# xxxupeng/stereo_toolbox

Hardware: AMD Instinct MI355X
Metric: stereo pairs/sec @ 540x960 D=192 (GwcNet_GC fwd+bwd) (higher is better)
Workload: dtype f32; 1 GPU; GwcNet_GC(maxdisp=192) train step: fwd+bwd+allreduce+Adam, 576x960 pairs (reference pad_to_2x shape), batch 1/GPU, fp32, synthetic randn inputs, deterministic filler weights; global_batch=1, parallelism=dp1, grad_sync=none (single rank: flat fp32 buffer packed, no collective), launch=eager, optimizer=torch.optim.Adam(fused=True)

## Files before the change

### include/stx_hip.h

```cpp
#ifndef STX_HIP_H
#define STX_HIP_H
#ifdef __cplusplus
extern "C" {
#endif

const char* stx_last_error(void);
const char* stx_build_info(void);
int stx_get_tuning(const char* name);
int stx_set_tuning(const char* name, int value);

int stx_cost_volume_fwd(const float* Lg, const float* Rg, int Cg, int G, const float* Lc, const float* Rc, int Cc,
                        const float* scale, float* vol, int B, int H, int W, int D, int mask_left, void* stream);
int stx_group_normalize_fwd(const float* x, float* y, int B, int C, int G, int HW, float out_scale, void* stream);
int stx_group_normalize_bwd(const float* x, const float* gy, float* gx, int B, int C, int G, int HW, float out_scale, void* stream);
int stx_cost_volume_bwd(const float* gvol, const float* Lg, const float* Rg, int Cg, int G, int Cc, float* gLg,
                        float* gRg, float* gLc, float* gRc, int B, int H, int W, int D, int mask_left, void* stream);

int stx_head_fwd(const float* cost, float* disp, float* stats, int B, int Dc, int Hc, int Wc, int D, int H, int W,
                 void* stream);
long long stx_head_bwd_workspace_floats(int B, int Dc, int H, int W);
int stx_head_bwd(const float* gdisp, const float* cost, const float* disp, const float* stats, float* gcost,
                 float* workspace, int B, int Dc, int Hc, int Wc, int D, int H, int W, void* stream);
int stx_head_fwd2(const float* cost, float* disp, float* stats, int B, int Dc, int Hc, int Wc, int D, int H, int W,
                  int align_corners, void* stream);
// ... 27 lines not shown
int stx_conv3d_wgrad_bn(const float* x, const float* gy, const float* z, const float* scale, const float* shift, const float* mean,
                        const float* invstd, const float* gamma, const float* sums, float inv_n, int act, float* dz, float* dw,
                        float* workspace, int B, int D, int H, int W, int CF, int CC, void* stream);

int stx_conv2d_supported(int Cin, int Cout);
long long stx_conv2d_stat_rows(int groups);
int stx_conv2d_fwd(const float* x, const float* w, float* out, float* stats, int B, int H, int W, int Cin, int Cout, int dgrad,
                   int groups, void* stream);

int stx_conv3d_c1_fwd(const float* x, const float* w, const float* residual, float* out, int B, int D, int H, int W,
                      int Cin, void* stream);
long long stx_conv3d_c1_wgrad_workspace_floats(int Cin);
int stx_conv3d_c1_wgrad(const float* x, const float* gy, float* dw, float* workspace, int B, int D, int H, int W,
                        int Cin, void* stream);
int stx_conv3d_c1_dgrad(const float* gy, const float* w, float* gx, int B, int D, int H, int W, int Cin, void* stream);

int stx_mish_fwd(const float* x, float* y, long long n, void* stream);
int stx_mish_bwd(const float* gy, const float* x, float* gx, long long n, void* stream);
int stx_depth_to_space(const float* y, float* out, int B, int D, int H, int W, int C, int inverse, void* stream);
int stx_gate_fwd(const float* cv, const float* att, float* out, int B, int D, long long HW, int C, void* stream);
int stx_gate_bwd(const float* g, const float* cv, const float* att, float* gcv, float* gatt, int B, int D, long long HW,
                 int C, void* stream);

int stx_concat_channels(const float* in0, const float* in1, const float* in2, const float* in3, int C0, int C1, int C2, int C3,
                        float* out, long long nvox, void* stream);
int stx_split_channels(const float* in, float* out0, float* out1, float* out2, float* out3, int C0, int C1, int C2, int C3,
                       long long nvox, void* stream);
int stx_transpose(const float* in, float* out, int N, int rows, int cols, void* stream);

int stx_dwconv_hw_fwd(const float* x, const float* w, const int* dil, float* out, int B, int D, int H, int W, int C,
// ... 175 lines not shown
```

### stereo_toolbox_amd/_capi.py

```python
import ctypes
import os
import threading

import torch

_P = ctypes.c_void_p
_I = ctypes.c_int
_F = ctypes.c_float
_L = ctypes.c_longlong

SIGNATURES = {
    "stx_get_tuning": [ctypes.c_char_p],
    "stx_set_tuning": [ctypes.c_char_p, _I],
    "stx_cost_volume_fwd": [_P, _P, _I, _I, _P, _P, _I, _P, _P, _I, _I, _I, _I, _I, _P],
    "stx_cost_volume_bwd": [_P, _P, _P, _I, _I, _I, _P, _P, _P, _P, _I, _I, _I, _I, _I, _P],
    "stx_group_normalize_fwd": [_P, _P, _I, _I, _I, _I, _F, _P],
    "stx_group_normalize_bwd": [_P, _P, _P, _I, _I, _I, _I, _F, _P],
    "stx_head_fwd": [_P, _P, _P, _I, _I, _I, _I, _I, _I, _I, _P],
    "stx_head_bwd_workspace_floats": [_I, _I, _I, _I],
    "stx_head_bwd": [_P, _P, _P, _P, _P, _P, _I, _I, _I, _I, _I, _I, _I, _P],
    "stx_head_fwd2": [_P, _P, _P, _I, _I, _I, _I, _I, _I, _I, _I, _P],
    "stx_head_bwd2": [_P, _P, _P, _P, _P, _P, _I, _I, _I, _I, _I, _I, _I, _I, _P],
    "stx_softargmax_fwd": [_P, _P, _I, _I, _I, _P],
    "stx_argmax_fwd": [_P, _P, _I, _I, _I, _P],
# ... 9 lines not shown
    "stx_conv3d_fwd_stat_rows": [_I, _I, _I, _I, _I, _I, _I, _I],
    "stx_deconv3d_fwd_blocks": [_I, _I, _I],
    "stx_conv3d_fwd": [_P, _P, _P, _P, _P, _P, _P, _I, _I, _I, _I, _I, _I, _I, _I, _I, _P],
    "stx_deconv3d_fwd": [_P, _P, _P, _P, _P, _P, _P, _I, _I, _I, _I, _I, _I, _I, _I, _I, _I, _P],
    "stx_conv3d_wgrad_workspace_floats": [_I, _I, _I, _I, _I, _I, _I, _I],
    "stx_conv3d_wgrad": [_P, _P, _P, _P, _I, _I, _I, _I, _I, _I, _I, _I, _I, _I, _I, _P],
    "stx_conv3d_wgrad_bn_supported": [_I, _I, _I, _I, _I, _I],
    "stx_conv3d_wgrad_bn": [_P] * 9 + [_F, _I, _P, _P, _P, _I, _I, _I, _I, _I, _I, _P],
    "stx_conv2d_supported": [_I, _I],
    "stx_conv2d_stat_rows": [_I],
    "stx_conv2d_fwd": [_P, _P, _P, _P, _I, _I, _I, _I, _I, _I, _I, _P],
    "stx_conv3d_c1_fwd": [_P, _P, _P, _P, _I, _I, _I, _I, _I, _P],
    "stx_conv3d_c1_wgrad_workspace_floats": [_I],
    "stx_conv3d_c1_wgrad": [_P, _P, _P, _P, _I, _I, _I, _I, _I, _P],
    "stx_conv3d_c1_dgrad": [_P, _P, _P, _I, _I, _I, _I, _I, _P],
    "stx_mish_fwd": [_P, _P, _L, _P],
    "stx_mish_bwd": [_P, _P, _P, _L, _P],
    "stx_depth_to_space": [_P, _P, _I, _I, _I, _I, _I, _I, _P],
    "stx_gate_fwd": [_P, _P, _P, _I, _I, _L, _I, _P],
    "stx_gate_bwd": [_P, _P, _P, _P, _P, _I, _I, _L, _I, _P],
    "stx_concat_channels": [_P, _P, _P, _P, _I, _I, _I, _I, _P, _L, _P],
    "stx_split_channels": [_P, _P, _P, _P, _P, _I, _I, _I, _I, _L, _P],
    "stx_transpose": [_P, _P, _I, _I, _I, _P],
    "stx_dwconv_hw_fwd": [_P, _P, _P, _P, _I, _I, _I, _I, _I, _I, _P],
    "stx_dwconv_hw_wgrad_workspace_floats": [_I],
    "stx_dwconv_hw_wgrad": [_P, _P, _P, _P, _P, _I, _I, _I, _I, _I, _P],
    "stx_cost_volume_scale_bwd": [_P, _P, _P, _P, _I, _I, _I, _I, _I, _I, _P],
    "stx_scale_channels": [_P, _P, _P, _L, _I, _P],
    "stx_ac_volume_bwd": [_P, _P, _P, _P, _P, _P, _P, _I, _I, _I, _I, _I, _I, _P],
    "stx_pad_normalize_u8": [_P, _P, _I, _I, _I, _I, _I, _I, _P, _P, _P],
# ... 144 lines not shown
```

### stereo_toolbox_amd/aggregation.py

```python
import os
import threading

import torch
import torch.nn as nn

from . import ops


def _is_transposed(conv):
    return isinstance(conv, nn.ConvTranspose3d)


def _conv_cfg(conv):
    ks = conv.kernel_size[0]
    stride = conv.stride[0]
    if _is_transposed(conv):
        k3 = ks == 3 and stride == 2 and conv.padding[0] == 1 and conv.output_padding[0] == 1
        k4 = ks == 4 and stride == 2 and conv.padding[0] == 1 and conv.output_padding[0] == 0
        if not (k3 or k4) or len(set(conv.kernel_size)) != 1 or len(set(conv.stride)) != 1:
            raise ops.StxError("only ConvTranspose3d(k=3, s=2, p=1, op=1) and ConvTranspose3d(k=4, s=2, p=1) are on the hot path")
    else:
        if not ((ks == 3 and conv.padding[0] == 1 and stride in (1, 2)) or (ks == 1 and conv.padding[0] == 0 and stride == 1)):
            raise ops.StxError(f"unsupported Conv3d k={ks} s={stride} p={conv.padding}")
    if conv.bias is not None or conv.groups != 1:
# ... 164 lines not shown
    if bn is None:
        y = z1
        if residual is not None:
            y = y + residual
        if relu == 3:
            return torch.nn.functional.leaky_relu(y, 0.01)
        return torch.relu(y) if relu else y
    count1 = z1.numel() // z1.shape[-1]
    st1 = _bn_state(bn, part1 if want else None, count1)
    if second is not None:
        x2, conv2, bn2 = second
        want2 = bn2.training
        z2, part2 = second_raw if second_raw is not None else _raw_conv(x2, conv2, want2)
        st2 = _bn_state(bn2, part2 if want2 else None, z2.numel() // z2.shape[-1])
        return ops.BnActFn.apply(z1, bn.weight, bn.bias, z2, bn2.weight, bn2.bias, None, relu, st1, st2)
    defer = (residual is None and want and relu in (0, 1, False, True) and not _is_transposed(conv) and _conv_cfg(conv) == (3, 1)
             and conv.weight.shape[0] % 32 == 0 and conv.weight.shape[1] % 32 == 0 and not st1.get("sync")
             and os.environ.get("STX_BN_BWD_IN_WGRAD", "1") != "0")
    if defer:
        ops.bn_defer_reset_if_stale()
    return ops.BnActFn.apply(z1, bn.weight, bn.bias, None, None, None, residual, relu, st1, None, 1, defer)


@ops.fp32_region
def convbn_block(x, seq, relu=False, second=None, residual=None, mish=False, raw=None, second_raw=None):
    sec = None
    if second is not None:
        sec = (second[0], second[1][0], second[1][1])
    return conv_block(x, seq[0], seq[1], relu=relu, second=sec, residual=residual, mish=mish, raw=raw, second_raw=second_raw)
```

### stereo_toolbox_amd/csrc/conv_c1.hip

```cpp
#include "stx_common.h"
#include <stdlib.h>

namespace {

constexpr int C1_THREADS = 256;
constexpr int C1_TD = 2, C1_TH = 4, C1_TW = 32;
constexpr int C1_ED = C1_TD + 2, C1_EH = C1_TH + 2, C1_EW = C1_TW + 2;
constexpr int C1_CK = 16, C1_VS = C1_CK + 4;

struct C1Args {
    const float* x;
    const float* w;
    const float* gy;
    const float* res;
    float* out;
    int B, D, H, W, Cin;
    int nDt, nHt, nWt, ntiles;
};

__device__ __forceinline__ void c1_stage(const C1Args& a, float* tile, int b, int d0, int h0, int w0, int c0, int tid) {
    for (int idx = tid; idx < C1_ED * C1_EH * C1_EW * (C1_CK / 4); idx += C1_THREADS) {
        const int v = idx / (C1_CK / 4), f = idx - v * (C1_CK / 4);
        const int wx = v % C1_EW, hy = (v / C1_EW) % C1_EH, dz = v / (C1_EW * C1_EH);
        const int gd = d0 - 1 + dz, gh = h0 - 1 + hy, gw = w0 - 1 + wx;
// ... 228 lines not shown
        const unsigned vbase = (unsigned)((((oh < H ? oh : 0) * W + w0 + 4 * half) * 32 + i) * 4);
#pragma unroll
        for (int r = 0; r < 16; ++r) {
            const int m = (r & 3) + 8 * (r >> 2);
            const bool ok = oh < H && w0 + 4 * half + m < W;
            stx_buf_st1(ors, ok ? vbase : STX_BUF_OOB, (unsigned)(m * 128), acc[r]);
        }
    }
}


constexpr int C1M_TD = 2, C1M_TH = 8, C1M_TW = 32;
constexpr int C1M_ED = C1M_TD + 2, C1M_EH = C1M_TH + 2, C1M_EW = C1M_TW + 2;
constexpr int C1M_BLOCKS = 1024;

__global__ __launch_bounds__(C1_THREADS) void conv_c1_wgrad_mfma_kernel(const float* __restrict__ x,
                                                                        const float* __restrict__ gy,
                                                                        float* __restrict__ slab, int B, int D, int H,
                                                                        int W, int Cin, int nDt, int nHt, int nWt,
                                                                        int ntiles) {
    __shared__ float gys[C1M_ED * C1M_EH * C1M_EW];
    __shared__ float red[4][1024];
    const int tid = threadIdx.x, lane = tid & 63, wave = tid >> 6;
    const int i = lane & 31, half = lane >> 5;
    const int cb = blockIdx.y;
    const int kd = i / 9, kh = (i / 3) % 3, kw = i % 3;
    const int toff = (i < 27) ? ((2 - kd) * C1M_EH + (2 - kh)) * C1M_EW + (2 - kw) + half : half;
    f32x16 acc;
#pragma unroll
    for (int r = 0; r < 16; ++r) acc[r] = 0.f;
    for (int t = blockIdx.x; t < ntiles; t += gridDim.x) {
        int r = t;
        const int wt = r % nWt; r /= nWt;
        const int ht = r % nHt; r /= nHt;
        const int dt = r % nDt;
        const int b = r / nDt;
        const int d0 = dt * C1M_TD, h0 = ht * C1M_TH, w0 = wt * C1M_TW;
        __syncthreads();
        for (int idx = tid; idx < C1M_ED * C1M_EH * C1M_EW; idx += C1_THREADS) {
            const int wx = idx % C1M_EW, hy = (idx / C1M_EW) % C1M_EH, dz = idx / (C1M_EW * C1M_EH);
            const int gd = d0 - 1 + dz, gh = h0 - 1 + hy, gw = w0 - 1 + wx;
            gys[idx] = (gd >= 0 && gd < D && gh >= 0 && gh < H && gw >= 0 && gw < W)
                           ? gy[(((size_t)b * D + gd) * H + gh) * W + gw] : 0.f;
        }
        __syncthreads();
#pragma unroll 1
        for (int k = 0; k < 4; ++k) {
            const int row = wave * 4 + k;
            const int ld = row / C1M_TH, lh = row % C1M_TH;
            const int gd = d0 + ld, gh = h0 + lh;
            const bool rowok = gd < D && gh < H;
            const float* xr = x + ((((size_t)b * D + gd) * H + gh) * W + w0 + half) * Cin + cb * 32 + i;
            float av[16];
#pragma unroll
            for (int p = 0; p < 16; ++p)
                av[p] = (rowok && w0 + 2 * p + half < W) ? xr[(size_t)(2 * p) * Cin] : 0.f;
            const float* gp = gys + (ld * C1M_EH + lh) * C1M_EW + toff;
#pragma unroll
            for (int p = 0; p < 16; ++p) {
                float bv = gp[2 * p];
                bv = (i < 27) ? bv : 0.f;
                acc = __builtin_amdgcn_mfma_f32_32x32x2f32(av[p], bv, acc, 0, 0, 0);
            }
        }
    }
#pragma unroll
    for (int r = 0; r < 16; ++r) red[wave][((r & 3) + 8 * (r >> 2) + 4 * half) * 32 + i] = acc[r];
    __syncthreads();
    float* dst = slab + ((size_t)cb * gridDim.x + blockIdx.x) * 1024;
    for (int idx = tid; idx < 1024; idx += C1_THREADS)
        dst[idx] = (red[0][idx] + red[1][idx]) + (red[2][idx] + red[3][idx]);
// ... 10 lines not shown
    red[tid] = s;
    __syncthreads();
    for (int k = C1_THREADS / 2; k > 0; k >>= 1) {
        if (tid < k) red[tid] += red[tid + k];
        __syncthreads();
    }
    if (tid == 0) dw[m] = (float)red[0];
}


constexpr int C1F_TH = 8, C1F_TW = 32;
constexpr int C1F_EH = C1F_TH + 2, C1F_EW = C1F_TW + 2, C1F_NV = C1F_EH * C1F_EW;
constexpr int C1F_MT = (C1F_NV + 31) / 32;
constexpr int C1F_WGS = 512;

__global__ __launch_bounds__(C1_THREADS) void conv_c1_fwd_mfma_kernel(const float* __restrict__ x,
                                                                      const float* __restrict__ w,
                                                                      const float* __restrict__ res,
                                                                      float* __restrict__ out, int B, int D, int H, int W,
                                                                      int nHt, int nWt, int ncols) {
    STX_DYN_SMEM(smem);
    float* Ps = reinterpret_cast<float*>(smem);
    const int tid = threadIdx.x, lane = tid & 63, wave = __builtin_amdgcn_readfirstlane(tid >> 6);
    const int i = lane & 31, half = lane >> 5;
    float wreg[16];
#pragma unroll
    for (int s_ = 0; s_ < 16; ++s_) wreg[s_] = (i < 27) ? w[(size_t)(16 * half + s_) * 27 + i] : 0.f;
    const int lh = tid / C1F_TW, lw = tid % C1F_TW;

    constexpr int MTW = (C1F_MT + 3) / 4;
    const long long units = (long long)ncols * D;
    int u = __builtin_amdgcn_readfirstlane((int)(units * blockIdx.x / gridDim.x));
    const int u_end = __builtin_amdgcn_readfirstlane((int)(units * (blockIdx.x + 1) / gridDim.x));
    const unsigned plane_bytes = (unsigned)H * (unsigned)W * 32u * 4u;
    while (u < u_end) {
        const int col = u / D;
        const int d_lo = u - col * D;
        const int left = u_end - u;
        const int d_hi = (D - d_lo < left) ? D : d_lo + left;
        u += d_hi - d_lo;
        const int wt = col % nWt, ht = (col / nWt) % nHt, b = col / (nWt * nHt);
        const int h0 = ht * C1F_TH, w0 = wt * C1F_TW;
// ... 22 lines not shown
        __syncthreads();
        for (int p = d_lo - 1; p <= d_hi; ++p) {
            float* Pb = Ps + ((p + 2) & 1) * (C1F_NV * 27);
            const bool pin = p >= 0 && p < D;
            float4 cur[MTW][4];
#pragma unroll
            for (int t = 0; t < MTW; ++t)
#pragma unroll
                for (int q = 0; q < 4; ++q) cur[t][q] = nxt[t][q];
            load_plane(p + 1);
            if (pin) {
#pragma unroll
                for (int t = 0; t < MTW; ++t) {
                    const int m = wave + 4 * t;
                    if (m < C1F_MT) {
                        f32x16 acc;
#pragma unroll
                        for (int r = 0; r < 16; ++r) acc[r] = 0.f;
#pragma unroll
                        for (int q = 0; q < 4; ++q) {
                            acc = __builtin_amdgcn_mfma_f32_32x32x2f32(cur[t][q].x, wreg[4 * q + 0], acc, 0, 0, 0);
                            acc = __builtin_amdgcn_mfma_f32_32x32x2f32(cur[t][q].y, wreg[4 * q + 1], acc, 0, 0, 0);
                            acc = __builtin_amdgcn_mfma_f32_32x32x2f32(cur[t][q].z, wreg[4 * q + 2], acc, 0, 0, 0);
                            acc = __builtin_amdgcn_mfma_f32_32x32x2f32(cur[t][q].w, wreg[4 * q + 3], acc, 0, 0, 0);
                        }
                        if (i < 27) {
#pragma unroll
                            for (int r = 0; r < 16; ++r) {
                                const int v = m * 32 + (r & 3) + 8 * (r >> 2) + 4 * half;
                                if (v < C1F_NV) Pb[v * 27 + i] = acc[r];
// ... 17 lines not shown
            }
            const float done = accA + s2;
            const int od = p - 1;
            if (od >= d_lo && od < d_hi && ook) {
                const size_t o = (((size_t)b * D + od) * H + oh) * W + ow;
                out[o] = res ? done + res[o] : done;
            }
            accA = accB + s1;
            accB = s0;
        }
    }
}

}

extern "C" int stx_conv3d_c1_fwd(const float* x, const float* w, const float* residual, float* out, int B, int D,
                                 int H, int W, int Cin, void* stream) {
    stx_begin();
    STX_REQUIRE(x && w && out && B > 0 && D > 0 && H > 0 && W > 0, "conv3d_c1_fwd: bad shape");
    STX_REQUIRE(Cin % C1_CK == 0, "conv3d_c1_fwd: Cin=%d must be a multiple of %d", Cin, C1_CK);
    if (Cin == 32 && (long long)H * W * 128 < (1ll << 31)) {
        const int nHt = stx_cdiv(H, C1F_TH), nWt = stx_cdiv(W, C1F_TW);
        const long long ncols = (long long)B * nHt * nWt, units = ncols * D;
        STX_REQUIRE(units < (1ll << 31), "conv3d_c1_fwd: volume too large");
        long long g = C1F_WGS;
        if (g > units / 4) g = units / 4 > 0 ? units / 4 : 1;
        const size_t lds = (size_t)2 * C1F_NV * 27 * 4;
        if (int rc = stx_lds_require((const void*)conv_c1_fwd_mfma_kernel, lds, "conv3d_c1_fwd(mfma)")) return rc;
        hipLaunchKernelGGL(conv_c1_fwd_mfma_kernel, dim3((unsigned)g), dim3(C1_THREADS), lds, (hipStream_t)stream, x, w,
                           residual, out, B, D, H, W, nHt, nWt, (int)ncols);
        return stx_check_launch("conv3d_c1_fwd(mfma)");
    }
    C1Args a;
    a.x = x; a.w = w; a.gy = nullptr; a.res = residual; a.out = out;
    a.B = B; a.D = D; a.H = H; a.W = W; a.Cin = Cin;
    a.nDt = stx_cdiv(D, C1_TD); a.nHt = stx_cdiv(H, C1_TH); a.nWt = stx_cdiv(W, C1_TW);
    a.ntiles = B * a.nDt * a.nHt * a.nWt;
    if (int rc = stx_lds_require((const void*)conv_c1_fwd_kernel, C1_TILE_BYTES, "conv3d_c1_fwd")) return rc;
    hipLaunchKernelGGL(conv_c1_fwd_kernel, dim3(a.ntiles), dim3(C1_THREADS), C1_TILE_BYTES, (hipStream_t)stream, a);
    return stx_check_launch("conv3d_c1_fwd");
}

extern "C" long long stx_conv3d_c1_wgrad_workspace_floats(int Cin) {
    const long long valu = (long long)C1_WGRAD_BLOCKS * Cin * 27;
    const long long mfma = (long long)C1M_BLOCKS * 1024 * ((Cin + 31) / 32);
    return valu > mfma ? valu : mfma;
}

extern "C" int stx_conv3d_c1_wgrad(const float* x, const float* gy, float* dw, float* workspace, int B, int D, int H,
                                   int W, int Cin, void* stream) {
    stx_begin();
    STX_REQUIRE(x && gy && dw && workspace && B > 0, "conv3d_c1_wgrad: null operand");
    STX_REQUIRE(Cin % C1_CK == 0 && Cin <= 4 * C1_CK, "conv3d_c1_wgrad: Cin=%d must be 16..64 in steps of 16", Cin);
    if (Cin % 32 == 0) {
        const int nDt = stx_cdiv(D, C1M_TD), nHt = stx_cdiv(H, C1M_TH), nWt = stx_cdiv(W, C1M_TW);
        const long long nt = (long long)B * nDt * nHt * nWt;
        STX_REQUIRE(nt < (1ll << 31), "conv3d_c1_wgrad: volume too large");
        const int nblk = nt < C1M_BLOCKS ? (int)nt : C1M_BLOCKS;
        hipStream_t st = (hipStream_t)stream;
        hipLaunchKernelGGL(conv_c1_wgrad_mfma_kernel, dim3(nblk, Cin / 32), dim3(C1_THREADS), 0, st, x, gy, workspace, B,
                           D, H, W, Cin, nDt, nHt, nWt, (int)nt);
        int rc = stx_check_launch("conv3d_c1_wgrad(mfma)");
        if (rc) return rc;
        hipLaunchKernelGGL(c1m_reduce_kernel, dim3(Cin * 27), dim3(C1_THREADS), 0, st, workspace, nblk, dw);
        return stx_check_launch("conv3d_c1_wgrad(reduce)");
    }
    C1Args a;
    a.x = x; a.w = nullptr; a.gy = gy; a.res = nullptr; a.out = workspace;
    a.B = B; a.D = D; a.H = H; a.W = W; a.Cin = Cin;
    a.nDt = stx_cdiv(D, C1_TD); a.nHt = stx_cdiv(H, C1_TH); a.nWt = stx_cdiv(W, C1_TW);
    a.ntiles = B * a.nDt * a.nHt * a.nWt;
    const int nblk = a.ntiles < C1_WGRAD_BLOCKS ? a.ntiles : C1_WGRAD_BLOCKS;
    const size_t lds = C1_TILE_BYTES + 256 * 4;
    hipStream_t st = (hipStream_t)stream;
    if (int rc = stx_lds_require((const void*)conv_c1_wgrad_kernel, lds, "conv3d_c1_wgrad")) return rc;
    hipLaunchKernelGGL(conv_c1_wgrad_kernel, dim3(nblk), dim3(C1_THREADS), lds, st, a);
    if (int rc = stx_check_launch("conv3d_c1_wgrad")) return rc;
    hipLaunchKernelGGL(c1_colsum_kernel, dim3(Cin * 27), dim3(C1_THREADS), 0, st, workspace, nblk, Cin * 27, dw);
    return stx_check_launch("conv3d_c1_colsum");
}

extern "C" int stx_conv3d_c1_dgrad(const float* gy, const float* w, float* gx, int B, int D, int H, int W, int Cin,
                                   void* stream) {
    stx_begin();
    STX_REQUIRE(gy && w && gx && B > 0 && D > 0 && H > 0 && W > 0, "conv3d_c1_dgrad: bad shape");
    STX_REQUIRE(Cin % 4 == 0 && Cin <= 64, "conv3d_c1_dgrad: Cin=%d must be a multiple of 4, <= 64", Cin);
    const int nHt = stx_cdiv(H, C1D_TH), nWt = stx_cdiv(W, C1D_TW);
    const long long nt = (long long)B * D * nHt * nWt;
    if (Cin == 32 && (long long)H * W * 128 < (1ll << 31) && nt < (1ll << 31)) {
        const long long g = nt < 256 * 8 ? nt : 256 * 8;
        hipLaunchKernelGGL(conv_c1_dgrad_mfma_kernel, dim3((unsigned)g), dim3(C1_THREADS), 0, (hipStream_t)stream, gy, w, gx, B, D,
                           H, W, nHt, nWt, (int)nt);
        return stx_check_launch("conv3d_c1_dgrad(mfma)");
    }
    hipLaunchKernelGGL(conv_c1_dgrad_kernel, dim3((unsigned)((size_t)B * D * nHt * nWt)), dim3(C1_THREADS), 0,
                       (hipStream_t)stream, gy, w, gx, B, D, H, W, Cin, nHt, nWt);
// ... 3 lines not shown
```

### stereo_toolbox_amd/models/GwcNet/gwcnet.py

```python
import torch
import torch.nn as nn

from ... import ops
from ...aggregation import conv_block, convbn_block, deferred_bn_counters, shared_input_convs
from ..features2d import ResTrunk, cat_features, channels_last_weights_, convbn, init_reference_style, run_head2d, run_pair
from .submodule import convbn_3d


class feature_extraction(ResTrunk):
    fused_everywhere = True

    def __init__(self, concat_feature=False, concat_feature_channel=12):
        super().__init__()
        self.concat_feature = concat_feature
        if concat_feature:
            self.lastconv = nn.Sequential(convbn(320, 128, 3, 1, 1, 1), nn.ReLU(inplace=True),
                                          nn.Conv2d(128, concat_feature_channel, 1, bias=False))

    def forward(self, x):
        gwc = cat_features(self.trunk(x))
        if not self.concat_feature:
            return {"gwc_feature": gwc}
        return {"gwc_feature": gwc, "concat_feature": run_head2d(self.lastconv, gwc)}

# ... 22 lines not shown
        c3 = convbn_block(c2, self.conv3[0], relu=True, raw=r2[0])
        c4 = convbn_block(c3, self.conv4[0], relu=True)
        if mid is not None:
            c4 = mid(c4)
        c5 = convbn_block(c4, self.conv5, relu=True, second=(c2, self.redir2), second_raw=r2[1])
        out = convbn_block(c5, self.conv6, relu=True, second=(x, self.redir1), second_raw=rx[1])
        return (out, rx[2]) if also is not None else out


def classifier(c):
    return nn.Sequential(convbn_3d(c, c, 3, 1, 1), nn.ReLU(inplace=True),
                         nn.Conv3d(c, 1, kernel_size=3, padding=1, stride=1, bias=False))


def run_classifier(seq, x, add=None, raw=None):
    h = convbn_block(x, seq[0], relu=True, raw=raw)
    cost = conv_block(h, seq[2], residual=None if add is None else add.unsqueeze(-1))
    return cost.squeeze(-1)


class GwcNet(nn.Module):
    def __init__(self, maxdisp, use_concat_volume=False):
        super().__init__()
        self.maxdisp = maxdisp
        self.use_concat_volume = use_concat_volume
        self.num_groups = 40
        if use_concat_volume:
            self.concat_channels = 12
            self.feature_extraction = feature_extraction(True, self.concat_channels)
        else:
            self.concat_channels = 0
            self.feature_extraction = feature_extraction(False)
# ... 46 lines not shown
```

### stereo_toolbox_amd/ops.py

```python
import ctypes

import torch

from ._capi import StxError, get_lib

_P = ctypes.c_void_p


class _DevPtr(ctypes.c_void_p):
    """A device pointer that remembers the device of the tensor it came from: _call() reads the launch device off its
    own arguments, so nothing survives between launches (an exception between building the arguments and the launch
    cannot leak state into the next one)."""


def _stream(dev=None):
    return _P(torch.cuda.current_stream(dev).cuda_stream)


def _p(t):
    if t is None:
        return None
    p = _DevPtr(t.data_ptr())
    p.dev = t.device
    return p
# ... 719 lines not shown
    dist.all_reduce(tot, group=group)
    hi = tot.float()
    lo = (tot - hi.double()).float()
    return torch.stack((hi, lo)).contiguous(), count * world


@fp32_region
def bn_apply(z1, scale1, shift1, z2=None, scale2=None, shift2=None, relu=False, groups=1):
    out = torch.empty_like(z1)
    C = z1.shape[-1]
    _call("stx_bn_apply", _p(z1), _p(scale1), _p(shift1), _p(z2), _p(scale2), _p(shift2), _p(out),
          z1.numel() // C // groups, C, int(relu), groups)
    return out


class BnActFn(torch.autograd.Function):

    @staticmethod
    def forward(ctx, z1, gamma1, beta1, z2, gamma2, beta2, residual, relu, bn1, bn2, groups=1, defer=False):
        G = int(groups)
        ctx.defer = bool(defer)

        def affine(gamma, beta, bn):
            if bn["training"]:
                partials, count = bn["partials"], bn["count"]
                if bn.get("sync"):
                    if G > 1:
                        raise StxError("BnActFn: SyncBatchNorm with groups is not wired (SyncBN runs the views separately)")
                    partials, count = _sync_bn_partials(partials, count, *bn["sync"])
                return bn_finalize(partials, count, gamma, beta, bn["running_mean"], bn["running_var"], bn["momentum"],
                                   bn["eps"], G)
            invstd = torch.rsqrt(bn["running_var"] + bn["eps"])
            scale = gamma * invstd
            res = (scale, beta - bn["running_mean"] * scale, bn["running_mean"].clone(), invstd)
            return res if G == 1 else [t.unsqueeze(0).expand(G, -1).contiguous() for t in res]

        relu = int(relu)
        if relu == 2 and residual is not None:
            raise StxError("BnActFn: Mish with a plain residual is not wired (no model of the family uses it)")
        if G < 1 or z1.shape[0] % G:
            raise StxError(f"BnActFn: leading axis {z1.shape[0]} does not split into {G} groups")
        sc1, sh1, m1, i1 = affine(gamma1, beta1, bn1)
        two = z2 is not None
        if two:
            sc2, sh2, m2, i2 = affine(gamma2, beta2, bn2)
            y = bn_apply(z1, sc1, sh1, z2, sc2, sh2, relu, G)
        else:
            sc2 = sh2 = m2 = i2 = None
            y = bn_apply(z1, sc1, sh1, residual, None, None, relu, G)
        ctx.relu, ctx.two, ctx.has_res, ctx.groups = relu, two, residual is not None, G
        ctx.train1 = bn1["training"]
        ctx.train2 = bn2["training"] if two else False
        ctx.sync = bn1.get("sync") or (bn2.get("sync") if two else None)
        ctx.remask = bool(relu) and residual is None
        keep_y = y if (relu and not ctx.remask) else None
        ctx.save_for_backward(z1, gamma1, m1, i1, z2, gamma2, m2, i2, keep_y, sc1 if ctx.remask else None,
                              sh1 if ctx.remask else None, sc2 if (ctx.remask and two) else None,
                              sh2 if (ctx.remask and two) else None)
        return y

    @staticmethod
    def backward(ctx, gy):
        z1, gamma1, m1, i1, z2, gamma2, m2, i2, y, sc1, sh1, sc2, sh2 = ctx.saved_tensors
        gy = gy.contiguous()
        G = ctx.groups
        C = z1.shape[-1]
        nvox = z1.numel() // C // G
        lib = get_lib()
        NB = lib.raw("stx_bn_reduce_blocks")()
        part = _WS.get("bnred", G * NB * 3 * C, z1.device)
        sums_all = torch.empty(G + (1 if G > 1 else 0), 3, C, dtype=torch.float32, device=z1.device)
        sums = sums_all[:G]
        _call("stx_bn_bwd_reduce2", _p(gy), _p(y), _p(z1), _p(m1), _p(i1), _p(z2) if ctx.two else None,
              _p(m2) if ctx.two else None, _p(i2) if ctx.two else None, _p(sc1), _p(sh1), _p(sc2), _p(sh2), _p(part),
              _p(sums_all), nvox, C, int(ctx.relu), G)
        if not ctx.needs_input_grad[0] and not ctx.two and not ctx.has_res:
            tot = sums_all[G] if G > 1 else sums_all[0]
            return (None, tot[1], tot[0], None, None, None, None, None, None, None, None, None)
        if (ctx.defer and not ctx.two and not ctx.has_res and ctx.relu in (0, 1) and ctx.train1 and not ctx.sync and G == 1
                and (not ctx.relu or ctx.remask)):
            alias = gy.view_as(gy)
            pend = _PendingBn()
            pend.g, pend.z, pend.scale, pend.shift, pend.mean, pend.invstd = alias, z1, sc1, sh1, m1, i1
            pend.gamma, pend.sums, pend.inv_n, pend.act = gamma1, sums, 1.0 / nvox, int(ctx.relu)
            if pend.scale is None:
                pend.scale = pend.shift = m1
            _defer_pending_bn(alias, pend)
            tot = sums_all[0]
            return (alias, tot[1], tot[0], None, None, None, None, None, None, None, None, None)
        dz1 = torch.empty_like(z1)
        dz2 = torch.empty_like(z2) if ctx.two else None
        gres = torch.empty_like(z1) if (ctx.has_res and ctx.relu) else None
        use = sums
        if ctx.sync:
            import torch.distributed as dist
            use = sums.clone()
            dist.all_reduce(use, group=ctx.sync[0])
            use /= ctx.sync[1]
        if not ctx.train1 or (ctx.two and not ctx.train2):
            use = torch.zeros_like(sums)
        _call("stx_bn_bwd_apply2", _p(gy), _p(y), _p(z1), _p(m1), _p(i1), _p(gamma1), _p(z2) if ctx.two else None,
              _p(m2) if ctx.two else None, _p(i2) if ctx.two else None, _p(gamma2) if ctx.two else None, _p(sc1), _p(sh1),
              _p(sc2), _p(sh2), _p(use), _p(dz1), _p(dz2), _p(gres), nvox, C, int(ctx.relu), G)
        if ctx.has_res and not ctx.relu:
            gres = gy
        tot = sums_all[G] if G > 1 else sums_all[0]
        return (dz1, tot[1], tot[0], dz2, tot[2] if ctx.two else None, tot[0].clone() if ctx.two else None, gres,
                None, None, None, None, None)


class MishFn(torch.autograd.Function):

    @staticmethod
    def forward(ctx, x):
        x = x.contiguous()
        _chk(x, "x")
        y = torch.empty_like(x)
        _call("stx_mish_fwd", _p(x), _p(y), x.numel())
        ctx.save_for_backward(x)
        return y

    @staticmethod
    def backward(ctx, gy):
# ... 1740 lines not shown
```

Baseline: 0.1786 pairs/s.

## Fuse classifier BatchNorm+ReLU into the Conv3d(32,1) forward and weight-grad kernels

Adds BN-aware variants of the Cin=32 single-output 3D conv forward and weight-gradient MFMA kernels. They apply the BN affine transform and ReLU while loading the raw conv output, so the normalized activation tensor is never written. A new autograd function routes the GwcNet classifier through this path and reuses the shared BN backward helper, including the deferred-BN path. This removes one full-volume write and read per classifier in forward and backward, at the cost of recomputing the affine+ReLU inside each kernel and a more complex autograd path.

```diff
diff --git a/include/stx_hip.h b/include/stx_hip.h
--- a/include/stx_hip.h
+++ b/include/stx_hip.h
@@ -65,6 +65,10 @@
 int stx_conv3d_c1_wgrad(const float* x, const float* gy, float* dw, float* workspace, int B, int D, int H, int W,
                         int Cin, void* stream);
 int stx_conv3d_c1_dgrad(const float* gy, const float* w, float* gx, int B, int D, int H, int W, int Cin, void* stream);
+int stx_conv3d_c1_fwd_bn(const float* z, const float* scale, const float* shift, const float* w, const float* residual,
+                         float* out, int B, int D, int H, int W, int Cin, int act, void* stream);
+int stx_conv3d_c1_wgrad_bn(const float* z, const float* scale, const float* shift, const float* gy, float* dw,
+                           float* workspace, int B, int D, int H, int W, int Cin, int act, void* stream);
 
 int stx_mish_fwd(const float* x, float* y, long long n, void* stream);
 int stx_mish_bwd(const float* gy, const float* x, float* gx, long long n, void* stream);
diff --git a/stereo_toolbox_amd/_capi.py b/stereo_toolbox_amd/_capi.py
--- a/stereo_toolbox_amd/_capi.py
+++ b/stereo_toolbox_amd/_capi.py
@@ -47,6 +47,8 @@
     "stx_conv3d_c1_wgrad_workspace_floats": [_I],
     "stx_conv3d_c1_wgrad": [_P, _P, _P, _P, _I, _I, _I, _I, _I, _P],
     "stx_conv3d_c1_dgrad": [_P, _P, _P, _I, _I, _I, _I, _I, _P],
+    "stx_conv3d_c1_fwd_bn": [_P, _P, _P, _P, _P, _P, _I, _I, _I, _I, _I, _I, _P],
+    "stx_conv3d_c1_wgrad_bn": [_P, _P, _P, _P, _P, _P, _I, _I, _I, _I, _I, _I, _P],
     "stx_mish_fwd": [_P, _P, _L, _P],
     "stx_mish_bwd": [_P, _P, _P, _L, _P],
     "stx_depth_to_space": [_P, _P, _I, _I, _I, _I, _I, _I, _P],
diff --git a/stereo_toolbox_amd/aggregation.py b/stereo_toolbox_amd/aggregation.py
--- a/stereo_toolbox_amd/aggregation.py
+++ b/stereo_toolbox_amd/aggregation.py
@@ -202,12 +202,42 @@
         z2, part2 = second_raw if second_raw is not None else _raw_conv(x2, conv2, want2)
         st2 = _bn_state(bn2, part2 if want2 else None, z2.numel() // z2.shape[-1])
         return ops.BnActFn.apply(z1, bn.weight, bn.bias, z2, bn2.weight, bn2.bias, None, relu, st1, st2)
-    defer = (residual is None and want and relu in (0, 1, False, True) and not _is_transposed(conv) and _conv_cfg(conv) == (3, 1)
-             and conv.weight.shape[0] % 32 == 0 and conv.weight.shape[1] % 32 == 0 and not st1.get("sync")
-             and os.environ.get("STX_BN_BWD_IN_WGRAD", "1") != "0")
+    defer = _bn_defer_ok(conv, st1, relu, residual)
     if defer:
         ops.bn_defer_reset_if_stale()
     return ops.BnActFn.apply(z1, bn.weight, bn.bias, None, None, None, residual, relu, st1, None, 1, defer)
+
+
+def _bn_defer_ok(conv, st, relu, residual=None):
+    return (residual is None and st["training"] and relu in (0, 1, False, True) and not _is_transposed(conv)
+            and _conv_cfg(conv) == (3, 1) and conv.weight.shape[0] % 32 == 0 and conv.weight.shape[1] % 32 == 0
+            and not st.get("sync") and os.environ.get("STX_BN_BWD_IN_WGRAD", "1") != "0")
+
+
+@ops.fp32_region
+def classifier_tail(x, seq, tail, raw=None):
+    conv, bn = seq[0], seq[1]
+    if os.environ.get("STX_C1_BN_ONLOAD", "1") == "0":
+        return None
+    if not (isinstance(bn, nn.BatchNorm3d) and not isinstance(bn, nn.SyncBatchNorm) and bn.training
+            and bn.weight is not None and bn.bias is not None):
+        return None
+    if not (isinstance(tail, nn.Conv3d) and not _is_transposed(tail) and tail.bias is None and tail.groups == 1
+            and tuple(tail.weight.shape) == (1, 32, 3, 3, 3) and tail.stride == (1, 1, 1) and tail.padding == (1, 1, 1)
+            and conv.weight.shape[0] == 32 and not _is_transposed(conv)):
+        return None
+    if x.dtype != torch.float32 or x.shape[2] * x.shape[3] * 128 >= 1 << 31:
+        return None
+    if not (torch.is_grad_enabled() and (raw is not None or _needs_grad(x, conv, bn, tail))):
+        return None
+    z, part = raw if raw is not None else _raw_conv(x, conv, True)
+    if z.shape[-1] != 32 or z.shape[2] * z.shape[3] * 128 >= 1 << 31:
+        raise ops.StxError(f"classifier_tail: raw output {tuple(z.shape)} does not feed Conv3d(32, 1, 3)")
+    st = _bn_state(bn, part, z.numel() // z.shape[-1])
+    defer = _bn_defer_ok(conv, st, True)
+    if defer:
+        ops.bn_defer_reset_if_stale()
+    return ops.BnActC1Fn.apply(z, bn.weight, bn.bias, tail.weight, st, 1, defer)
 
 
 @ops.fp32_region
diff --git a/stereo_toolbox_amd/csrc/conv_c1.hip b/stereo_toolbox_amd/csrc/conv_c1.hip
--- a/stereo_toolbox_amd/csrc/conv_c1.hip
+++ b/stereo_toolbox_amd/csrc/conv_c1.hip
@@ -7,6 +7,11 @@
 constexpr int C1_TD = 2, C1_TH = 4, C1_TW = 32;
 constexpr int C1_ED = C1_TD + 2, C1_EH = C1_TH + 2, C1_EW = C1_TW + 2;
 constexpr int C1_CK = 16, C1_VS = C1_CK + 4;
+
+__device__ __forceinline__ float c1_bn_act(float z, float scale, float shift, bool pass, bool in) {
+    const float v = fmaf(z, scale, shift);
+    return (in & (pass | (v > 0.f))) ? v : 0.f;
+}
 
 struct C1Args {
     const float* x;
@@ -266,11 +271,13 @@
 constexpr int C1M_ED = C1M_TD + 2, C1M_EH = C1M_TH + 2, C1M_EW = C1M_TW + 2;
 constexpr int C1M_BLOCKS = 1024;
 
+template <bool BN>
 __global__ __launch_bounds__(C1_THREADS) void conv_c1_wgrad_mfma_kernel(const float* __restrict__ x,
                                                                         const float* __restrict__ gy,
                                                                         float* __restrict__ slab, int B, int D, int H,
                                                                         int W, int Cin, int nDt, int nHt, int nWt,
-                                                                        int ntiles) {
+                                                                        int ntiles, const float* __restrict__ scale,
+                                                                        const float* __restrict__ shift, int act) {
     __shared__ float gys[C1M_ED * C1M_EH * C1M_EW];
     __shared__ float red[4][1024];
     const int tid = threadIdx.x, lane = tid & 63, wave = tid >> 6;
@@ -278,6 +285,8 @@
     const int cb = blockIdx.y;
     const int kd = i / 9, kh = (i / 3) % 3, kw = i % 3;
     const int toff = (i < 27) ? ((2 - kd) * C1M_EH + (2 - kh)) * C1M_EW + (2 - kw) + half : half;
+    float bsc = 0.f, bsh = 0.f;
+    if constexpr (BN) { bsc = scale[cb * 32 + i]; bsh = shift[cb * 32 + i]; }
     f32x16 acc;
 #pragma unroll
     for (int r = 0; r < 16; ++r) acc[r] = 0.f;
@@ -307,6 +316,11 @@
 #pragma unroll
             for (int p = 0; p < 16; ++p)
                 av[p] = (rowok && w0 + 2 * p + half < W) ? xr[(size_t)(2 * p) * Cin] : 0.f;
+            if constexpr (BN) {
+#pragma unroll
+                for (int p = 0; p < 16; ++p)
+                    av[p] = c1_bn_act(av[p], bsc, bsh, act != 1, rowok && w0 + 2 * p + half < W);
+            }
             const float* gp = gys + (ld * C1M_EH + lh) * C1M_EW + toff;
 #pragma unroll
             for (int p = 0; p < 16; ++p) {
@@ -347,11 +361,14 @@
 constexpr int C1F_MT = (C1F_NV + 31) / 32;
 constexpr int C1F_WGS = 512;
 
+template <bool BN>
 __global__ __launch_bounds__(C1_THREADS) void conv_c1_fwd_mfma_kernel(const float* __restrict__ x,
                                                                       const float* __restrict__ w,
                                                                       const float* __restrict__ res,
                                                                       float* __restrict__ out, int B, int D, int H, int W,
-                                                                      int nHt, int nWt, int ncols) {
+                                                                      int nHt, int nWt, int ncols,
+                                                                      const float* __restrict__ scale,
+                                                                      const float* __restrict__ shift, int act) {
     STX_DYN_SMEM(smem);
     float* Ps = reinterpret_cast<float*>(smem);
     const int tid = threadIdx.x, lane = tid & 63, wave = __builtin_amdgcn_readfirstlane(tid >> 6);
@@ -359,6 +376,11 @@
     float wreg[16];
 #pragma unroll
     for (int s_ = 0; s_ < 16; ++s_) wreg[s_] = (i < 27) ? w[(size_t)(16 * half + s_) * 27 + i] : 0.f;
+    float bsc[16], bsh[16];
+    if constexpr (BN) {
+#pragma unroll
+        for (int s_ = 0; s_ < 16; ++s_) { bsc[s_] = scale[16 * half + s_]; bsh[s_] = shift[16 * half + s_]; }
+    }
     const int lh = tid / C1F_TW, lw = tid % C1F_TW;
 
     constexpr int MTW = (C1F_MT + 3) / 4;
@@ -411,6 +433,17 @@
                 for (int t = 0; t < MTW; ++t) {
                     const int m = wave + 4 * t;
                     if (m < C1F_MT) {
+                        if constexpr (BN) {
+                            const bool vok = voff[t] != STX_BUF_OOB, pass = act != 1;
+#pragma unroll
+                            for (int q = 0; q < 4; ++q) {
+                                float4& c4 = cur[t][q];
+                                c4.x = c1_bn_act(c4.x, bsc[4 * q + 0], bsh[4 * q + 0], pass, vok);
+                                c4.y = c1_bn_act(c4.y, bsc[4 * q + 1], bsh[4 * q + 1], pass, vok);
+                                c4.z = c1_bn_act(c4.z, bsc[4 * q + 2], bsh[4 * q + 2], pass, vok);
+                                c4.w = c1_bn_act(c4.w, bsc[4 * q + 3], bsh[4 * q + 3], pass, vok);
+                            }
+                        }
                         f32x16 acc;
 #pragma unroll
                         for (int r = 0; r < 16; ++r) acc[r] = 0.f;
@@ -458,23 +491,44 @@
 
 }
 
+template <bool BN>
+static int c1_fwd_mfma_launch(const float* x, const float* scale, const float* shift, int act, const float* w,
+                              const float* residual, float* out, int B, int D, int H, int W, void* stream) {
+    const int nHt = stx_cdiv(H, C1F_TH), nWt = stx_cdiv(W, C1F_TW);
+    const long long ncols = (long long)B * nHt * nWt, units = ncols * D;
+    STX_REQUIRE(units < (1ll << 31), "conv3d_c1_fwd: volume too large");
+    long long g = C1F_WGS;
+    if (g > units / 4) g = units / 4 > 0 ? units / 4 : 1;
+    const size_t lds = (size_t)2 * C1F_NV * 27 * 4;
+    if (int rc = stx_lds_require((const void*)conv_c1_fwd_mfma_kernel<BN>, lds, "conv3d_c1_fwd(mfma)")) return rc;
+    hipLaunchKernelGGL(conv_c1_fwd_mfma_kernel<BN>, dim3((unsigned)g), dim3(C1_THREADS), lds, (hipStream_t)stream, x, w,
+                       residual, out, B, D, H, W, nHt, nWt, (int)ncols, scale, shift, act);
+    return stx_check_launch("conv3d_c1_fwd(mfma)");
+}
+
+template <bool BN>
+static int c1_wgrad_mfma_launch(const float* x, const float* scale, const float* shift, int act, const float* gy, float* dw,
+                                float* workspace, int B, int D, int H, int W, int Cin, void* stream) {
+    const int nDt = stx_cdiv(D, C1M_TD), nHt = stx_cdiv(H, C1M_TH), nWt = stx_cdiv(W, C1M_TW);
+    const long long nt = (long long)B * nDt * nHt * nWt;
+    STX_REQUIRE(nt < (1ll << 31), "conv3d_c1_wgrad: volume too large");
+    const int nblk = nt < C1M_BLOCKS ? (int)nt : C1M_BLOCKS;
+    hipStream_t st = (hipStream_t)stream;
+    hipLaunchKernelGGL(conv_c1_wgrad_mfma_kernel<BN>, dim3(nblk, Cin / 32), dim3(C1_THREADS), 0, st, x, gy, workspace, B,
+                       D, H, W, Cin, nDt, nHt, nWt, (int)nt, scale, shift, act);
+    int rc = stx_check_launch("conv3d_c1_wgrad(mfma)");
+    if (rc) return rc;
+    hipLaunchKernelGGL(c1m_reduce_kernel, dim3(Cin * 27), dim3(C1_THREADS), 0, st, workspace, nblk, dw);
+    return stx_check_launch("conv3d_c1_wgrad(reduce)");
+}
+
 extern "C" int stx_conv3d_c1_fwd(const float* x, const float* w, const float* residual, float* out, int B, int D,
                                  int H, int W, int Cin, void* stream) {
     stx_begin();
     STX_REQUIRE(x && w && out && B > 0 && D > 0 && H > 0 && W > 0, "conv3d_c1_fwd: bad shape");
     STX_REQUIRE(Cin % C1_CK == 0, "conv3d_c1_fwd: Cin=%d must be a multiple of %d", Cin, C1_CK);
-    if (Cin == 32 && (long long)H * W * 128 < (1ll << 31)) {
-        const int nHt = stx_cdiv(H, C1F_TH), nWt = stx_cdiv(W, C1F_TW);
-        const long long ncols = (long long)B * nHt * nWt, units = ncols * D;
-        STX_REQUIRE(units < (1ll << 31), "conv3d_c1_fwd: volume too large");
-        long long g = C1F_WGS;
-        if (g > units / 4) g = units / 4 > 0 ? units / 4 : 1;
-        const size_t lds = (size_t)2 * C1F_NV * 27 * 4;
-        if (int rc = stx_lds_require((const void*)conv_c1_fwd_mfma_kernel, lds, "conv3d_c1_fwd(mfma)")) return rc;
-        hipLaunchKernelGGL(conv_c1_fwd_mfma_kernel, dim3((unsigned)g), dim3(C1_THREADS), lds, (hipStream_t)stream, x, w,
-                           residual, out, B, D, H, W, nHt, nWt, (int)ncols);
-        return stx_check_launch("conv3d_c1_fwd(mfma)");
-    }
+    if (Cin == 32 && (long long)H * W * 128 < (1ll << 31))
+        return c1_fwd_mfma_launch<false>(x, nullptr, nullptr, 0, w, residual, out, B, D, H, W, stream);
     C1Args a;
     a.x = x; a.w = w; a.gy = nullptr; a.res = residual; a.out = out;
     a.B = B; a.D = D; a.H = H; a.W = W; a.Cin = Cin;
@@ -485,6 +539,16 @@
     return stx_check_launch("conv3d_c1_fwd");
 }
 
+extern "C" int stx_conv3d_c1_fwd_bn(const float* z, const float* scale, const float* shift, const float* w,
+                                    const float* residual, float* out, int B, int D, int H, int W, int Cin, int act,
+                                    void* stream) {
+    stx_begin();
+    STX_REQUIRE(z && scale && shift && w && out && B > 0 && D > 0 && H > 0 && W > 0, "conv3d_c1_fwd_bn: bad shape");
+    STX_REQUIRE(Cin == 32 && (act == 0 || act == 1), "conv3d_c1_fwd_bn: Cin=%d act=%d (serves Cin = 32, act 0 / 1)", Cin, act);
+    STX_REQUIRE((long long)H * W * 128 < (1ll << 31), "conv3d_c1_fwd_bn: plane beyond the descriptor range");
+    return c1_fwd_mfma_launch<true>(z, scale, shift, act, w, residual, out, B, D, H, W, stream);
+}
+
 extern "C" long long stx_conv3d_c1_wgrad_workspace_floats(int Cin) {
     const long long valu = (long long)C1_WGRAD_BLOCKS * Cin * 27;
     const long long mfma = (long long)C1M_BLOCKS * 1024 * ((Cin + 31) / 32);
@@ -496,19 +560,8 @@
     stx_begin();
     STX_REQUIRE(x && gy && dw && workspace && B > 0, "conv3d_c1_wgrad: null operand");
     STX_REQUIRE(Cin % C1_CK == 0 && Cin <= 4 * C1_CK, "conv3d_c1_wgrad: Cin=%d must be 16..64 in steps of 16", Cin);
-    if (Cin % 32 == 0) {
-        const int nDt = stx_cdiv(D, C1M_TD), nHt = stx_cdiv(H, C1M_TH), nWt = stx_cdiv(W, C1M_TW);
-        const long long nt = (long long)B * nDt * nHt * nWt;
-        STX_REQUIRE(nt < (1ll << 31), "conv3d_c1_wgrad: volume too large");
-        const int nblk = nt < C1M_BLOCKS ? (int)nt : C1M_BLOCKS;
-        hipStream_t st = (hipStream_t)stream;
-        hipLaunchKernelGGL(conv_c1_wgrad_mfma_kernel, dim3(nblk, Cin / 32), dim3(C1_THREADS), 0, st, x, gy, workspace, B,
-                           D, H, W, Cin, nDt, nHt, nWt, (int)nt);
-        int rc = stx_check_launch("conv3d_c1_wgrad(mfma)");
-        if (rc) return rc;
-        hipLaunchKernelGGL(c1m_reduce_kernel, dim3(Cin * 27), dim3(C1_THREADS), 0, st, workspace, nblk, dw);
-        return stx_check_launch("conv3d_c1_wgrad(reduce)");
-    }
+    if (Cin % 32 == 0)
+        return c1_wgrad_mfma_launch<false>(x, nullptr, nullptr, 0, gy, dw, workspace, B, D, H, W, Cin, stream);
     C1Args a;
     a.x = x; a.w = nullptr; a.gy = gy; a.res = nullptr; a.out = workspace;
     a.B = B; a.D = D; a.H = H; a.W = W; a.Cin = Cin;
@@ -524,6 +577,15 @@
     return stx_check_launch("conv3d_c1_colsum");
 }
 
+extern "C" int stx_conv3d_c1_wgrad_bn(const float* z, const float* scale, const float* shift, const float* gy, float* dw,
+                                      float* workspace, int B, int D, int H, int W, int Cin, int act, void* stream) {
+    stx_begin();
+    STX_REQUIRE(z && scale && shift && gy && dw && workspace && B > 0 && D > 0 && H > 0 && W > 0,
+                "conv3d_c1_wgrad_bn: null operand");
+    STX_REQUIRE(Cin == 32 && (act == 0 || act == 1), "conv3d_c1_wgrad_bn: Cin=%d act=%d (serves Cin = 32, act 0 / 1)", Cin, act);
+    return c1_wgrad_mfma_launch<true>(z, scale, shift, act, gy, dw, workspace, B, D, H, W, Cin, stream);
+}
+
 extern "C" int stx_conv3d_c1_dgrad(const float* gy, const float* w, float* gx, int B, int D, int H, int W, int Cin,
                                    void* stream) {
     stx_begin();
diff --git a/stereo_toolbox_amd/models/GwcNet/gwcnet.py b/stereo_toolbox_amd/models/GwcNet/gwcnet.py
--- a/stereo_toolbox_amd/models/GwcNet/gwcnet.py
+++ b/stereo_toolbox_amd/models/GwcNet/gwcnet.py
@@ -2,7 +2,7 @@
 import torch.nn as nn
 
 from ... import ops
-from ...aggregation import conv_block, convbn_block, deferred_bn_counters, shared_input_convs
+from ...aggregation import classifier_tail, conv_block, convbn_block, deferred_bn_counters, shared_input_convs
 from ..features2d import ResTrunk, cat_features, channels_last_weights_, convbn, init_reference_style, run_head2d, run_pair
 from .submodule import convbn_3d
 
@@ -60,8 +60,13 @@
 
 
 def run_classifier(seq, x, add=None, raw=None):
+    residual = None if add is None else add.unsqueeze(-1)
+    if isinstance(seq[1], nn.ReLU):
+        cost = classifier_tail(x, seq[0], seq[2], raw=raw)
+        if cost is not None:
+            return (cost if residual is None else cost + residual).squeeze(-1)
     h = convbn_block(x, seq[0], relu=True, raw=raw)
-    cost = conv_block(h, seq[2], residual=None if add is None else add.unsqueeze(-1))
+    cost = conv_block(h, seq[2], residual=residual)
     return cost.squeeze(-1)
 
 
diff --git a/stereo_toolbox_amd/ops.py b/stereo_toolbox_amd/ops.py
--- a/stereo_toolbox_amd/ops.py
+++ b/stereo_toolbox_amd/ops.py
@@ -757,36 +757,85 @@
     return out
 
 
+def _bn_affine(gamma, beta, bn, G=1):
+    if bn["training"]:
+        partials, count = bn["partials"], bn["count"]
+        if bn.get("sync"):
+            if G > 1:
+                raise StxError("BnActFn: SyncBatchNorm with groups is not wired (SyncBN runs the views separately)")
+            partials, count = _sync_bn_partials(partials, count, *bn["sync"])
+        return bn_finalize(partials, count, gamma, beta, bn["running_mean"], bn["running_var"], bn["momentum"],
+                           bn["eps"], G)
+    invstd = torch.rsqrt(bn["running_var"] + bn["eps"])
+    scale = gamma * invstd
+    res = (scale, beta - bn["running_mean"] * scale, bn["running_mean"].clone(), invstd)
+    return res if G == 1 else [t.unsqueeze(0).expand(G, -1).contiguous() for t in res]
+
+
+def _bn_act_backward(ctx, gy, need_dz1, saved):
+    z1, gamma1, m1, i1, z2, gamma2, m2, i2, y, sc1, sh1, sc2, sh2 = saved
+    gy = gy.contiguous()
+    G = ctx.groups
+    C = z1.shape[-1]
+    nvox = z1.numel() // C // G
+    lib = get_lib()
+    NB = lib.raw("stx_bn_reduce_blocks")()
+    part = _WS.get("bnred", G * NB * 3 * C, z1.device)
+    sums_all = torch.empty(G + (1 if G > 1 else 0), 3, C, dtype=torch.float32, device=z1.device)
+    sums = sums_all[:G]
+    _call("stx_bn_bwd_reduce2", _p(gy), _p(y), _p(z1), _p(m1), _p(i1), _p(z2) if ctx.two else None,
+          _p(m2) if ctx.two else None, _p(i2) if ctx.two else None, _p(sc1), _p(sh1), _p(sc2), _p(sh2), _p(part),
+          _p(sums_all), nvox, C, int(ctx.relu), G)
+    if not need_dz1 and not ctx.two and not ctx.has_res:
+        tot = sums_all[G] if G > 1 else sums_all[0]
+        return (None, tot[1], tot[0], None, None, None, None)
+    if (ctx.defer and not ctx.two and not ctx.has_res and ctx.relu in (0, 1) and ctx.train1 and not ctx.sync and G == 1
+            and (not ctx.relu or ctx.remask)):
+        alias = gy.view_as(gy)
+        pend = _PendingBn()
+        pend.g, pend.z, pend.scale, pend.shift, pend.mean, pend.invstd = alias, z1, sc1, sh1, m1, i1
+        pend.gamma, pend.sums, pend.inv_n, pend.act = gamma1, sums, 1.0 / nvox, int(ctx.relu)
+        if pend.scale is None:
+            pend.scale = pend.shift = m1
+        _defer_pending_bn(alias, pend)
+        tot = sums_all[0]
+        return (alias, tot[1], tot[0], None, None, None, None)
+    dz1 = torch.empty_like(z1)
+    dz2 = torch.empty_like(z2) if ctx.two else None
+    gres = torch.empty_like(z1) if (ctx.has_res and ctx.relu) else None
+    use = sums
+    if ctx.sync:
+        import torch.distributed as dist
+        use = sums.clone()
+        dist.all_reduce(use, group=ctx.sync[0])
+        use /= ctx.sync[1]
+    if not ctx.train1 or (ctx.two and not ctx.train2):
+        use = torch.zeros_like(sums)
+    _call("stx_bn_bwd_apply2", _p(gy), _p(y), _p(z1), _p(m1), _p(i1), _p(gamma1), _p(z2) if ctx.two else None,
+          _p(m2) if ctx.two else None, _p(i2) if ctx.two else None, _p(gamma2) if ctx.two else None, _p(sc1), _p(sh1),
+          _p(sc2), _p(sh2), _p(use), _p(dz1), _p(dz2), _p(gres), nvox, C, int(ctx.relu), G)
+    if ctx.has_res and not ctx.relu:
+        gres = gy
+    tot = sums_all[G] if G > 1 else sums_all[0]
+    return (dz1, tot[1], tot[0], dz2, tot[2] if ctx.two else None, tot[0].clone() if ctx.two else None, gres)
+
+
 class BnActFn(torch.autograd.Function):
 
     @staticmethod
     def forward(ctx, z1, gamma1, beta1, z2, gamma2, beta2, residual, relu, bn1, bn2, groups=1, defer=False):
         G = int(groups)
         ctx.defer = bool(defer)
-
-        def affine(gamma, beta, bn):
-            if bn["training"]:
-                partials, count = bn["partials"], bn["count"]
-                if bn.get("sync"):
-                    if G > 1:
-                        raise StxError("BnActFn: SyncBatchNorm with groups is not wired (SyncBN runs the views separately)")
-                    partials, count = _sync_bn_partials(partials, count, *bn["sync"])
-                return bn_finalize(partials, count, gamma, beta, bn["running_mean"], bn["running_var"], bn["momentum"],
-                                   bn["eps"], G)
-            invstd = torch.rsqrt(bn["running_var"] + bn["eps"])
-            scale = gamma * invstd
-            res = (scale, beta - bn["running_mean"] * scale, bn["running_mean"].clone(), invstd)
-            return res if G == 1 else [t.unsqueeze(0).expand(G, -1).contiguous() for t in res]
 
         relu = int(relu)
         if relu == 2 and residual is not None:
             raise StxError("BnActFn: Mish with a plain residual is not wired (no model of the family uses it)")
         if G < 1 or z1.shape[0] % G:
             raise StxError(f"BnActFn: leading axis {z1.shape[0]} does not split into {G} groups")
-        sc1, sh1, m1, i1 = affine(gamma1, beta1, bn1)
+        sc1, sh1, m1, i1 = _bn_affine(gamma1, beta1, bn1, G)
         two = z2 is not None
         if two:
-            sc2, sh2, m2, i2 = affine(gamma2, beta2, bn2)
+            sc2, sh2, m2, i2 = _bn_affine(gamma2, beta2, bn2, G)
             y = bn_apply(z1, sc1, sh1, z2, sc2, sh2, relu, G)
         else:
             sc2 = sh2 = m2 = i2 = None
@@ -804,52 +853,45 @@
 
     @staticmethod
     def backward(ctx, gy):
-        z1, gamma1, m1, i1, z2, gamma2, m2, i2, y, sc1, sh1, sc2, sh2 = ctx.saved_tensors
-        gy = gy.contiguous()
-        G = ctx.groups
-        C = z1.shape[-1]
-        nvox = z1.numel() // C // G
-        lib = get_lib()
-        NB = lib.raw("stx_bn_reduce_blocks")()
-        part = _WS.get("bnred", G * NB * 3 * C, z1.device)
-        sums_all = torch.empty(G + (1 if G > 1 else 0), 3, C, dtype=torch.float32, device=z1.device)
-        sums = sums_all[:G]
-        _call("stx_bn_bwd_reduce2", _p(gy), _p(y), _p(z1), _p(m1), _p(i1), _p(z2) if ctx.two else None,
-              _p(m2) if ctx.two else None, _p(i2) if ctx.two else None, _p(sc1), _p(sh1), _p(sc2), _p(sh2), _p(part),
-              _p(sums_all), nvox, C, int(ctx.relu), G)
-        if not ctx.needs_input_grad[0] and not ctx.two and not ctx.has_res:
-            tot = sums_all[G] if G > 1 else sums_all[0]
-            return (None, tot[1], tot[0], None, None, None, None, None, None, None, None, None)
-        if (ctx.defer and not ctx.two and not ctx.has_res and ctx.relu in (0, 1) and ctx.train1 and not ctx.sync and G == 1
-                and (not ctx.relu or ctx.remask)):
-            alias = gy.view_as(gy)
-            pend = _PendingBn()
-            pend.g, pend.z, pend.scale, pend.shift, pend.mean, pend.invstd = alias, z1, sc1, sh1, m1, i1
-            pend.gamma, pend.sums, pend.inv_n, pend.act = gamma1, sums, 1.0 / nvox, int(ctx.relu)
-            if pend.scale is None:
-                pend.scale = pend.shift = m1
-            _defer_pending_bn(alias, pend)
-            tot = sums_all[0]
-            return (alias, tot[1], tot[0], None, None, None, None, None, None, None, None, None)
-        dz1 = torch.empty_like(z1)
-        dz2 = torch.empty_like(z2) if ctx.two else None
-        gres = torch.empty_like(z1) if (ctx.has_res and ctx.relu) else None
-        use = sums
-        if ctx.sync:
-            import torch.distributed as dist
-            use = sums.clone()
-            dist.all_reduce(use, group=ctx.sync[0])
-            use /= ctx.sync[1]
-        if not ctx.train1 or (ctx.two and not ctx.train2):
-            use = torch.zeros_like(sums)
-        _call("stx_bn_bwd_apply2", _p(gy), _p(y), _p(z1), _p(m1), _p(i1), _p(gamma1), _p(z2) if ctx.two else None,
-              _p(m2) if ctx.two else None, _p(i2) if ctx.two else None, _p(gamma2) if ctx.two else None, _p(sc1), _p(sh1),
-              _p(sc2), _p(sh2), _p(use), _p(dz1), _p(dz2), _p(gres), nvox, C, int(ctx.relu), G)
-        if ctx.has_res and not ctx.relu:
-            gres = gy
-        tot = sums_all[G] if G > 1 else sums_all[0]
-        return (dz1, tot[1], tot[0], dz2, tot[2] if ctx.two else None, tot[0].clone() if ctx.two else None, gres,
-                None, None, None, None, None)
+        return _bn_act_backward(ctx, gy, ctx.needs_input_grad[0], ctx.saved_tensors) + (None, None, None, None, None)
+
+
+class BnActC1Fn(torch.autograd.Function):
+
+    @staticmethod
+    def forward(ctx, z, gamma, beta, w, bn, relu, defer):
+        _chk(z, "z", 5)
+        relu = int(relu)
+        B, D, H, W, C = z.shape
+        if (not bn["training"] or bn.get("sync") or relu not in (0, 1) or C != 32 or tuple(w.shape) != (1, 32, 3, 3, 3)
+                or H * W * 128 >= 1 << 31):
+            raise StxError("BnActC1Fn: serves a train-mode, unsynchronised BatchNorm3d(32) + ReLU / identity in front of "
+                           "Conv3d(32, 1, 3, padding=1) (aggregation.classifier_tail selects)")
+        sc, sh, m, i = _bn_affine(gamma, beta, bn)
+        wc = w.contiguous()
+        cost = torch.empty(B, D, H, W, 1, dtype=torch.float32, device=z.device)
+        _call("stx_conv3d_c1_fwd_bn", _p(z), _p(sc), _p(sh), _p(wc), None, _p(cost), B, D, H, W, C, relu)
+        ctx.relu, ctx.two, ctx.has_res, ctx.groups = relu, False, False, 1
+        ctx.train1, ctx.train2, ctx.sync, ctx.defer, ctx.remask = True, False, None, bool(defer), True
+        ctx.save_for_backward(z, gamma, m, i, sc, sh, wc)
+        return cost
+
+    @staticmethod
+    def backward(ctx, gcost):
+        z, gamma, m, i, sc, sh, w = ctx.saved_tensors
+        gcost = gcost.contiguous()
+        B, D, H, W, C = z.shape
+        gw = None
+        if ctx.needs_input_grad[3]:
+            ws = _WS.get("c1wgrad", get_lib().raw("stx_conv3d_c1_wgrad_workspace_floats")(C), z.device)
+            gw = torch.empty_like(w)
+            _call("stx_conv3d_c1_wgrad_bn", _p(z), _p(sc), _p(sh), _p(gcost), _p(gw), _p(ws), B, D, H, W, C, int(ctx.relu))
+        if not any(ctx.needs_input_grad[:3]):
+            return None, None, None, gw, None, None, None
+        gh = conv3d_c1_dgrad(gcost, w, C)
+        dz, dgamma, dbeta = _bn_act_backward(ctx, gh, ctx.needs_input_grad[0],
+                                             (z, gamma, m, i, None, None, None, None, None, sc, sh, None, None))[:3]
+        return dz, dgamma, dbeta, gw, None, None, None
 
 
 class MishFn(torch.autograd.Function):
```

New measurement: 0.1786 pairs/s. Within noise of the previous version (+0.0%).
